# CGuerreroCordova/HydroDEM

Measured on AMD Instinct MI355X. Metric: Mcells/s sink-fill+D8 on 16384^2 float32 DEM, higher is better.
Workload: dtype f32; 1 GPU; 16384x16384 float32 synthetic DEM (SURVEY 8d 'rough': plane + 4 sinusoids + 0.5 m noise + 0.1% pits), SinkFill eps=0 to exact convergence + D8; 16384 rows per GPU, row-block partition; rows_per_gpu=16384, cols=16384, tiles=70225, visits_unchanged=25936, visits_flat=3302, certifying_rounds=0, halo_exchanges=0

## Files before the change

hydrodem_amd/csrc/hdem_sinkfill.hip:

```cpp
#include "hdem_internal.h"

#include <algorithm>
#include <cmath>
#include <cstdlib>

namespace {

constexpr int FT = 62;
constexpr int WN = 64;
constexpr int TS = WN + 1;
constexpr int NT = 64;
constexpr int ITER_MAX = 8;
constexpr int INIT_NT = 256;
constexpr int INIT_ROWS = 4;
constexpr int KEY_NONE = 0x7fffffff;
constexpr int SEED_KEYS = 1 << 20;
constexpr int AUX_SC1 = 16;
constexpr int COARSE_SHIFT = 4;
constexpr int HUB_EDGE = 4 * WN;
constexpr float HUB_BIG = 3.0e38f;
constexpr int HUB_MIN_TILES = 64;
constexpr int HUB_MIN_TILES_NESTED = 36;
constexpr int COARSE_MIN_CELLS = 6000 * 6000;
constexpr int PEND_SHARDS = 64;
// ... 11 lines not shown
constexpr int HEAD_INTS = 32;
constexpr int FLAT_NONE = 0x7f7f7f7f;
enum { ST_IDLE = 0, ST_QUEUED = 1, ST_RUNNING = 2, ST_DIRTY = 3, ST_ROUND0 = 16 };

struct fill_ws {
    int *tile_key;
    int *state;
    int *prio;
    int *pend;
    int *any;
    int *error;
    unsigned long long *stats;
    int *flat;
    int *zmax;
    int *applied;
    int ntiles, tiles_x, tiles_y, max_rounds, G, S;
};

__device__ __forceinline__ float lane_prev(float v)
{
    return __builtin_bit_cast(float, __builtin_amdgcn_update_dpp(
        0, __builtin_bit_cast(int, v), 0x138, 0xF, 0xF, true));
}
__device__ __forceinline__ float lane_next(float v)
{
    return __builtin_bit_cast(float, __builtin_amdgcn_update_dpp(
        0, __builtin_bit_cast(int, v), 0x130, 0xF, 0xF, true));
}

__device__ __forceinline__ void or_changed(unsigned long long &acc, float a, float b)
{
    asm volatile("v_cmp_neq_f32 vcc, %1, %2\n\ts_or_b64 %0, %0, vcc"
                 : "+s"(acc) : "v"(a), "v"(b) : "vcc", "scc");
}
__device__ __forceinline__ void or_less(unsigned long long &acc, float a, float b)
{
    asm volatile("v_cmp_lt_f32 vcc, %1, %2\n\ts_or_b64 %0, %0, vcc"
                 : "+s"(acc) : "v"(a), "v"(b) : "vcc", "scc");
}

__device__ __forceinline__ void shift_in_less(unsigned &acc, float a, float b)
{
    asm volatile("v_cmp_lt_f32 vcc, %1, %2\n\t"
                 "v_addc_co_u32 %0, vcc, %0, %0, vcc"
                 : "+v"(acc) : "v"(a), "v"(b) : "vcc");
}

__device__ __forceinline__ void column_bits(unsigned &west, unsigned &east, float a, float b,
                                            int shift)
{
    unsigned t;
    asm volatile("v_cmp_lt_f32 vcc, %3, %4\n\t"
                 "s_and_b32 %2, vcc_lo, 1\n\t"
                 "s_lshl_b32 %2, %2, %5\n\t"
                 "s_or_b32 %0, %0, %2\n\t"
                 "s_lshr_b32 %2, vcc_hi, 31\n\t"
                 "s_lshl_b32 %2, %2, %5\n\t"
                 "s_or_b32 %1, %1, %2"
                 : "+s"(west), "+s"(east), "=&s"(t)
                 : "v"(a), "v"(b), "i"(shift)
                 : "vcc", "scc");
}

struct scan_masks {
    unsigned long long first, last, all;
};

template <bool HAS_EPS>
__device__ __forceinline__ void scan_lines(const float (&z)[WN], float (&w)[WN], float eps)
{
    float pf = w[0], pb = w[WN - 1];
    asm volatile("s_nop 1" : "+v"(pf), "+v"(pb));
#pragma unroll
    for (int k = 1; k <= WN - 2; ++k) {
        const int i = k, j = WN - 1 - k;
        float t1, t2, cf, cb, nf, nb;
        if (HAS_EPS)
            asm("v_min_f32_dpp %0, %6, %6 wave_shr:1 row_mask:0xf bank_mask:0xf bound_ctrl:0\n\t"
                "v_min_f32_dpp %1, %7, %7 wave_shr:1 row_mask:0xf bank_mask:0xf bound_ctrl:0\n\t"
                "v_min_f32_dpp %2, %6, %0 wave_shl:1 row_mask:0xf bank_mask:0xf bound_ctrl:0\n\t"
                "v_min_f32_dpp %3, %7, %1 wave_shl:1 row_mask:0xf bank_mask:0xf bound_ctrl:0\n\t"
                "v_add_f32 %2, %2, %12\n\t"
                "v_add_f32 %3, %3, %12\n\t"
                "v_med3_f32 %4, %8, %9, %2\n\t"
                "v_med3_f32 %5, %10, %11, %3"
                : "=&v"(t1), "=&v"(t2), "=&v"(cf), "=&v"(cb), "=&v"(nf), "=&v"(nb)
                : "v"(pf), "v"(pb), "v"(z[i]), "v"(w[i]), "v"(z[j]), "v"(w[j]), "v"(eps));
        else
            asm("v_min_f32_dpp %0, %6, %6 wave_shr:1 row_mask:0xf bank_mask:0xf bound_ctrl:0\n\t"
                "v_min_f32_dpp %1, %7, %7 wave_shr:1 row_mask:0xf bank_mask:0xf bound_ctrl:0\n\t"
                "v_min_f32_dpp %2, %6, %0 wave_shl:1 row_mask:0xf bank_mask:0xf bound_ctrl:0\n\t"
                "v_min_f32_dpp %3, %7, %1 wave_shl:1 row_mask:0xf bank_mask:0xf bound_ctrl:0\n\t"
                "v_med3_f32 %4, %8, %9, %2\n\t"
                "v_med3_f32 %5, %10, %11, %3"
                : "=&v"(t1), "=&v"(t2), "=&v"(cf), "=&v"(cb), "=&v"(nf), "=&v"(nb)
                : "v"(pf), "v"(pb), "v"(z[i]), "v"(w[i]), "v"(z[j]), "v"(w[j]));
        w[i] = nf;
        pf = nf;
        w[j] = nb;
        pb = nb;
    }
}

template <bool HAS_EPS>
__device__ __forceinline__ void check_rows(const float (&z)[WN], float (&w)[WN], float eps,
                                           scan_masks &m)
{
    float h_prev = fminf(fminf(w[0], lane_prev(w[0])), lane_next(w[0]));
    float h_cur = fminf(fminf(w[1], lane_prev(w[1])), lane_next(w[1]));
#pragma unroll
    for (int r = 1; r <= WN - 2; ++r) {
        const float h_next = fminf(fminf(w[r + 1], lane_prev(w[r + 1])), lane_next(w[r + 1]));
        float c = fminf(fminf(h_prev, h_cur), h_next);
        if (HAS_EPS) c = c + eps;
        const float n = __builtin_amdgcn_fmed3f(z[r], w[r], c);
        if (r == 1) or_changed(m.first, n, w[r]);
        else if (r == WN - 2) or_changed(m.last, n, w[r]);
        else or_changed(m.all, n, w[r]);
        w[r] = n;
        h_prev = h_cur;
        h_cur = h_next;
    }
}

__device__ __forceinline__ void transpose(float (&v)[WN], float *T, int lane)
{
#pragma unroll
    for (int i = 0; i < WN; ++i) T[i * TS + lane] = v[i];
    __syncthreads();
#pragma unroll
    for (int i = 0; i < WN; ++i) v[i] = T[lane * TS + i];
    __syncthreads();
}

__device__ __forceinline__ float wave_min(float v)
{
#pragma unroll
    for (int o = 32; o >= 1; o >>= 1) v = fminf(v, __shfl_xor(v, o));
    return v;
}

__device__ __forceinline__ int float_key(float f)
{
    int i = __builtin_bit_cast(int, f);
    return i ^ ((i >> 31) & 0x7fffffff);
}

#ifdef HDEM_VISIT_PROF
#define PROF_MARK(k) do { long long now_ = wall_clock64(); out.ticks[k] += now_ - tprof_; tprof_ = now_; } while (0)
#else
#define PROF_MARK(k) do { } while (0)
#endif

struct hub_bounds {
    float lv[9];
    bool mine;
};

struct visit_result {
#ifdef HDEM_VISIT_PROF
    long long ticks[6];
#endif
    bool changed;
    bool more;
    unsigned dirs;
    int iters;
    int flat_bits;
    int zmax_bits;
};

template <bool HAS_EPS, bool COHERENT>
__device__ __forceinline__ visit_result tile_visit(const float *__restrict__ zg, float *wg,
                                                   int H, int W, float eps, int ty, int tx,
                                                   float *T, uint8_t *d8 = nullptr,
                                                   float flat_level = HDEM_INF,
                                                   const hub_bounds *hb = nullptr)
{
    const int lane = threadIdx.x;
    const int y0 = ty * FT, x0 = tx * FT;
    const int x = x0 + lane;
#ifdef HDEM_VISIT_PROF
    const long long tprof_entry_ = wall_clock64();
#endif

    float z[WN], w[WN];
    const int xc = min(x, W - 1);
    float *wbase = wg + (size_t)y0 * W;
    const size_t wbytes = (size_t)(H - y0) * W * sizeof(float);
    const __amdgpu_buffer_rsrc_t wrsrc = __builtin_amdgcn_make_buffer_rsrc(
        wbase, 0, COHERENT ? (int)(unsigned)(wbytes < 0xffffffffull ? wbytes : 0xffffffffull) : 0,
        0x00020000);
    const int hbrow = H - 1 - y0;
    if (COHERENT) {
        const __amdgpu_buffer_rsrc_t zrsrc = __builtin_amdgcn_make_buffer_rsrc(
            const_cast<float *>(zg) + (size_t)y0 * W, 0,
            (int)(unsigned)(wbytes < 0xffffffffull ? wbytes : 0xffffffffull), 0x00020000);
        const unsigned col = (unsigned)xc * (unsigned)sizeof(float);
        const unsigned pitch = (unsigned)W * (unsigned)sizeof(float);
#pragma unroll
        for (int r = 0; r < WN; ++r) {
            const unsigned row = (unsigned)min(r, hbrow) * pitch;
            z[r] = __builtin_bit_cast(float, __builtin_amdgcn_raw_buffer_load_b32(zrsrc, col, row, 0));
            w[r] = __builtin_bit_cast(float, __builtin_amdgcn_raw_buffer_load_b32(wrsrc, col, row, AUX_SC1));
        }
    } else {
#pragma unroll
        for (int r = 0; r < WN; ++r) {
            const size_t o = (size_t)min(y0 + r, H - 1) * W + xc;
            z[r] = zg[o];
            w[r] = wg[o];
        }
    }
    const bool lane_pin = lane == 0 || lane == WN - 1 || x == 0 || x >= W - 1;
    const bool lane_out = x >= W;
    const bool partial = x0 + WN > W || y0 + WN > H;
    unsigned long long free_n = ~0ull, free_s = ~0ull;
    unsigned free_lo = 0, free_hi = 0;
    float hub_t = -HDEM_INF, hub_m = -HDEM_INF, hub_b = -HDEM_INF;
    if (COHERENT && hb) {
        const int k = lane == 0 ? 0 : (lane == WN - 1 ? 2 : 1);
        hub_t = k == 0 ? hb->lv[0] : (k == 1 ? hb->lv[1] : hb->lv[2]);
        hub_m = k == 0 ? hb->lv[3] : (k == 1 ? hb->lv[4] : hb->lv[5]);
        hub_b = k == 0 ? hb->lv[6] : (k == 1 ? hb->lv[7] : hb->lv[8]);
    }
    const int pin_from = lane_pin ? 0 : min(hbrow, WN - 1);
    const int raise_to = x >= W - 1 ? 0 : min(hbrow, WN);
#pragma unroll
    for (int r = 0; r < WN; ++r) {
        float wc = fminf(w[r], HDEM_INF), zc = fminf(z[r], HDEM_INF);
        if (COHERENT) {
            const float bound = r == 0 ? hub_t : (r == WN - 1 ? hub_b : hub_m);
            wc = fmaxf(wc, r < raise_to ? bound : -HDEM_INF);
        }
        if (!COHERENT && partial && (lane_out || y0 + r >= H)) { wc = HDEM_INF; zc = HDEM_INF; }
        if (COHERENT) {
            if (r == 0) free_n = __ballot(zc < wc);
            if (r == WN - 1) free_s = __ballot(zc < wc);
            if (r < 32) shift_in_less(free_lo, zc, wc);
            else shift_in_less(free_hi, zc, wc);
        }
        z[r] = (r == 0 || r == WN - 1 || r >= pin_from) ? wc : zc;
        w[r] = wc;
    }
    if (COHERENT && partial) {
        const unsigned long long in_lanes = __ballot(!lane_out);
        free_n &= in_lanes;
        free_s = hbrow >= WN - 1 ? (free_s & in_lanes) : 0ull;
    }

    if (COHERENT && flat_level < HDEM_INF) {
        const bool inner_lane = lane >= 2 && lane <= FT - 1;
#pragma unroll
        for (int r = 2; r <= FT - 1; ++r) w[r] = inner_lane ? flat_level : w[r];
    }

    unsigned long long free_w = 0, free_e = 0;
    if (COHERENT) {
        const unsigned wl = __builtin_amdgcn_readlane(free_lo, 0), wh = __builtin_amdgcn_readlane(free_hi, 0);
        const unsigned el = __builtin_amdgcn_readlane(free_lo, WN - 1), eh = __builtin_amdgcn_readlane(free_hi, WN - 1);
        free_w = ((unsigned long long)__builtin_bitreverse32(wh) << 32) | __builtin_bitreverse32(wl);
        free_e = ((unsigned long long)__builtin_bitreverse32(eh) << 32) | __builtin_bitreverse32(el);
        if (partial && hbrow < WN - 1) {
            const unsigned long long in_rows = (2ull << hbrow) - 1;
            free_w &= in_rows;
            free_e &= in_rows;
        }
    }
    visit_result out;
    out.flat_bits = out.zmax_bits = FLAT_NONE;
#ifdef HDEM_VISIT_PROF
    for (int k = 0; k < 6; ++k) out.ticks[k] = 0;
    long long tprof_ = tprof_entry_;
    asm volatile("s_waitcnt vmcnt(0)" ::: "memory");
    PROF_MARK(0);
#endif
    out.dirs = 0;
    out.iters = 0;
    scan_masks V = {0, 0, 0};
    check_rows<HAS_EPS>(z, w, eps, V);
    V.all |= V.first | V.last;
    bool more = V.all != 0;
    out.changed = more;
    const bool force_store = COHERENT && hb && hb->mine;
    const unsigned long long b1 = 1ull << 1, bl = 1ull << FT;
    unsigned long long mv_r1 = V.first, mv_r62 = V.last, mv_c1 = V.all & b1, mv_c62 = V.all & bl;
    PROF_MARK(1);
    if (more || force_store) {
        float zt[WN];
#pragma unroll
        for (int r = 0; r < WN; ++r) zt[r] = z[r];
        transpose(zt, T, lane);
        float r1_prev = w[1], r62_prev = w[FT];
        if (lane == 1 || lane == FT) {
            float *dst = T + (lane == 1 ? 0 : WN);
#pragma unroll
            for (int r = 0; r < WN; ++r) dst[r] = w[r];
        }
        __syncthreads();
        float c1_prev = T[lane], c62_prev = T[WN + lane];
        __syncthreads();
        float hl = HDEM_INF, hr = HDEM_INF;
        PROF_MARK(2);
        for (; out.iters < ITER_MAX && more; ++out.iters) {
            scan_lines<HAS_EPS>(z, w, eps);
            transpose(w, T, lane);
            hl = w[0];
            hr = w[WN - 1];
            or_changed(mv_c1, w[1], c1_prev);
            or_changed(mv_c62, w[FT], c62_prev);
            c1_prev = w[1];
            c62_prev = w[FT];
            scan_lines<HAS_EPS>(zt, w, eps);
            or_changed(mv_c1, w[1], c1_prev);
            or_changed(mv_c62, w[FT], c62_prev);
            c1_prev = w[1];
            c62_prev = w[FT];
#pragma unroll
            for (int i = 0; i < WN; ++i) T[lane * TS + i] = w[i];
            __syncthreads();
#pragma unroll
            for (int i = 0; i < WN; ++i) w[i] = T[i * TS + lane];
            __syncthreads();
            or_changed(mv_r1, w[1], r1_prev);
            or_changed(mv_r62, w[FT], r62_prev);
            scan_masks c = {0, 0, 0};
            check_rows<HAS_EPS>(z, w, eps, c);
            c.all |= c.first | c.last;
            mv_r1 |= c.first;
            mv_r62 |= c.last;
            mv_c1 |= c.all & b1;
            mv_c62 |= c.all & bl;
            r1_prev = w[1];
            r62_prev = w[FT];
            more = c.all != 0;
        }

        PROF_MARK(3);
        if (lane >= 1 && lane <= FT && x <= W - 2) {
#pragma unroll
            for (int r = 1; r <= FT; ++r) {
                const int y = y0 + r;
                if (y <= H - 2) {
                    const float val = z[r] == HDEM_INF ? __builtin_nanf("") : w[r];
                    if (COHERENT)
                        __builtin_amdgcn_raw_buffer_store_b32(
                            __builtin_bit_cast(unsigned, val), wrsrc,
                            (unsigned)(((size_t)r * W + x) * sizeof(float)), 0, AUX_SC1);
                    else
                        wg[(size_t)y * W + x] = val;
                }
            }
        }

#ifdef HDEM_VISIT_PROF
        asm volatile("s_waitcnt vmcnt(0)" ::: "memory");
#endif
        PROF_MARK(4);
        const unsigned long long mid = ((1ull << FT) - 1) << 1;
        const bool inner = lane >= 1 && lane <= FT;
        const float e1 = inner ? w[1] : HDEM_INF, e62 = inner ? w[FT] : HDEM_INF;
        const float p1s = lane_prev(e1), n1s = lane_next(e1);
        const float p62s = lane_prev(e62), n62s = lane_next(e62);
        const float p1 = lane == 0 ? HDEM_INF : p1s;
        const float n1 = lane == WN - 1 ? HDEM_INF : n1s;
        const float p62 = lane == 0 ? HDEM_INF : p62s;
        const float n62 = lane == WN - 1 ? HDEM_INF : n62s;
        float cn = fminf(fminf(e1, p1), n1), cs = fminf(fminf(e62, p62), n62);
        if (HAS_EPS) { cn += eps; cs += eps; }
        unsigned long long north = 0, south = 0;
        or_less(north, cn, w[0]);
        or_less(south, cs, w[WN - 1]);
        north &= free_n;
        south &= free_s;
        const bool row1_moved = mv_r1 != 0, row62_moved = mv_r62 != 0;
        if (row1_moved) {
            if (north & mid) out.dirs |= 1u << 1;
            if (north & 1ull) out.dirs |= 1u << 0;
            if (north & (1ull << (WN - 1))) out.dirs |= 1u << 2;
        }
        if (row62_moved) {
            if (south & mid) out.dirs |= 1u << 6;
            if (south & 1ull) out.dirs |= 1u << 5;
            if (south & (1ull << (WN - 1))) out.dirs |= 1u << 7;
        }
        const bool col1_moved = mv_c1 != 0, col62_moved = mv_c62 != 0;
        if (more) {
            if (col1_moved) out.dirs |= 1u << 3;
            if (col62_moved) out.dirs |= 1u << 4;
        } else if (col1_moved || col62_moved) {
            const float m1 = inner ? c1_prev : HDEM_INF, m62 = inner ? c62_prev : HDEM_INF;
            const float pws = lane_prev(m1), nxs = lane_next(m1);
            const float pes = lane_prev(m62), nes = lane_next(m62);
            const float pw = lane == 0 ? HDEM_INF : pws;
            const float nx = lane == WN - 1 ? HDEM_INF : nxs;
            const float pe = lane == 0 ? HDEM_INF : pes;
            const float ne = lane == WN - 1 ? HDEM_INF : nes;
            float cwest = fminf(fminf(m1, pw), nx), ceast = fminf(fminf(m62, pe), ne);
            if (HAS_EPS) { cwest += eps; ceast += eps; }
            unsigned long long west = 0, east = 0;
            or_less(west, cwest, hl);
            or_less(east, ceast, hr);
            if (COHERENT) {
                west &= free_w;
                east &= free_e;
            }
            if (col1_moved && (west & mid)) out.dirs |= 1u << 3;
            if (col62_moved && (east & mid)) out.dirs |= 1u << 4;
        }
        PROF_MARK(5);
    }
    if (COHERENT && !HAS_EPS && !partial && !more) {
        const bool inner_lane = lane >= 1 && lane <= FT;
        const float level = __builtin_bit_cast(
            float, __builtin_amdgcn_readlane(__builtin_bit_cast(int, w[31]), 31));
        if ((__ballot(inner_lane && w[31] != level) == 0) && level < HDEM_INF) {
            unsigned long long off = 0;
            float zm = -HDEM_INF;
#pragma unroll
            for (int r = 1; r <= FT; ++r) {
                or_changed(off, w[r], level);
                zm = fmaxf(zm, z[r]);
            }
            if ((off & ((((1ull << FT) - 1) << 1))) == 0) {
                zm = inner_lane ? zm : -HDEM_INF;
                zm = -wave_min(-zm);
                out.flat_bits = __builtin_bit_cast(int, level);
                out.zmax_bits = __builtin_bit_cast(int, zm);
            }
        }
    }
    if (!COHERENT && d8 && !out.changed) {
        const bool mine = lane >= 1 && lane <= FT && x <= W - 2;
        const float dg = 0.70710678f;
        float nw = lane_prev(w[0]), ne = lane_next(w[0]);
        float cw = lane_prev(w[1]), ce = lane_next(w[1]);
#pragma unroll
        for (int r = 1; r <= FT; ++r) {
            const float sw = lane_prev(w[r + 1]), se = lane_next(w[r + 1]);
            const float c = w[r];
            float best = 0.0f, d;
            unsigned code = 0;
            d = (c - nw) * dg;   if (d > best) { best = d; code = 32; }
            d = (c - w[r - 1]);  if (d > best) { best = d; code = 64; }
            d = (c - ne) * dg;   if (d > best) { best = d; code = 128; }
            d = (c - cw);        if (d > best) { best = d; code = 16; }
            d = (c - ce);        if (d > best) { best = d; code = 1; }
            d = (c - sw) * dg;   if (d > best) { best = d; code = 8; }
            d = (c - w[r + 1]);  if (d > best) { best = d; code = 4; }
            d = (c - se) * dg;   if (d > best) { best = d; code = 2; }
            if (z[r] == HDEM_INF) code = 0;
            const int y = y0 + r;
            if (mine && y <= H - 2) d8[(size_t)y * W + x] = (uint8_t)code;
            nw = cw; ne = ce; cw = sw; ce = se;
        }
    }
    out.more = more;
    return out;
}

__device__ __forceinline__ int neighbour_tile(int k, int ty, int tx, int tiles_x, int tiles_y)
{
    const int dy = k < 3 ? -1 : (k < 5 ? 0 : 1);
    const int dx = (k == 0 || k == 3 || k == 5) ? -1 : ((k == 1 || k == 6) ? 0 : 1);
    const int ny = ty + dy, nx = tx + dx;
    return (ny >= 0 && ny < tiles_y && nx >= 0 && nx < tiles_x) ? ny * tiles_x + nx : -1;
}

__device__ __forceinline__ void add_stats(unsigned long long *stats, int b, bool changed,
                                          bool more, int iters)
{
    unsigned long long *s = stats + (size_t)b * STAT_WORDS;
    s[0] += 1;
    s[1] += (unsigned long long)iters;
    s[2] += changed ? 0 : 1;
    s[3] += more ? 1 : 0;
}

template <bool HAS_EPS>
__global__ __launch_bounds__(NT, 2) void fill_round_kernel(const float *__restrict__ zg,
                                                          float *wg, int H, int W, float eps,
                                                          int tiles_x, int tiles_y, int ntiles,
                                                          int S, int *state, int stamp,
                                                          int *any_next,
                                                          unsigned long long *stats,
                                                          uint8_t *d8)
{
    __shared__ float T[WN * TS];
    const int lane = threadIdx.x;
    const int G = gridDim.x, b = blockIdx.x;
    int *my_state = state + (size_t)b * S;
    for (int base = 0; base < S; base += NT) {
        const int slot_l = base + lane;
        const bool due_l = slot_l < S && slot_l * G + b < ntiles && my_state[slot_l] == stamp;
        unsigned long long due = __ballot(due_l);
        while (due) {
            const int slot = base + __builtin_ctzll(due);
            due &= due - 1;
            const int t = slot * G + b;
            const int ty = t / tiles_x, tx = t - ty * tiles_x;
            visit_result v = tile_visit<HAS_EPS, false>(zg, wg, H, W, eps, ty, tx, T, d8);
            if (d8 && v.changed) { v.dirs = 0xffu; v.more = true; }
            if (lane < 8 && ((v.dirs >> lane) & 1u)) {
                const int t2 = neighbour_tile(lane, ty, tx, tiles_x, tiles_y);
                if (t2 >= 0) {
                    state[(size_t)(t2 % G) * S + t2 / G] = stamp + 1;
                    *any_next = 1;
                }
            }
            if (lane == 8) {
                if (v.more) {
                    my_state[slot] = stamp + 1;
                    *any_next = 1;
                }
                add_stats(stats, b, v.changed, v.more, v.iters);
                stats[(size_t)b * STAT_WORDS + 6] += 1;
#ifdef HDEM_VISIT_PROF
                for (int k = 0; k < 6; ++k) stats[(size_t)b * STAT_WORDS + STAT_PROF + k] += v.ticks[k];
#endif
            }
        }
    }
}

__device__ __forceinline__ int ld_relaxed(const int *p)
{
    return __hip_atomic_load(p, __ATOMIC_RELAXED, __HIP_MEMORY_SCOPE_AGENT);
}

__device__ __forceinline__ void wake_async(int t2, int key, int G, int S, int *state,
                                           int *prio, int *pend)
{
    const int owner = t2 % G, idx = owner * S + t2 / G;
    atomicMin(&prio[idx], key);
    for (int tries = 0; tries < 8; ++tries) {
        const int s = atomicCAS(&state[idx], ST_IDLE, ST_QUEUED);
        if (s == ST_IDLE) {
            atomicAdd(pend + (owner % PEND_SHARDS) * PEND_STRIDE, 1);
            return;
        }
        if (s == ST_QUEUED || s == ST_DIRTY) return;
        const int s2 = atomicCAS(&state[idx], ST_RUNNING, ST_DIRTY);
        if (s2 != ST_IDLE) return;
    }
}

__device__ __attribute__((noinline)) int async_pick(int b, int G, int S, int ntiles, int *state,
                                                    int *prio, const int *pend, int *error,
                                                    long long t_begin, long long budget_ticks)
{
    const int lane = threadIdx.x;
    int *my_state = state + (size_t)b * S, *my_prio = prio + (size_t)b * S;
    int zero_reads = 0;
    for (;;) {
        long long best = 0x7fffffffffffffffll;
        for (int base = 0; base < S; base += NT) {
            const int slot = base + lane;
            long long cand = 0x7fffffffffffffffll;
            if (slot < S && slot * G + b < ntiles && ld_relaxed(&my_state[slot]) == ST_QUEUED)
                cand = ((long long)ld_relaxed(&my_prio[slot]) << 32) | (unsigned)slot;
            best = cand < best ? cand : best;
        }
#pragma unroll
        for (int o = 32; o >= 1; o >>= 1) {
            const long long other = __shfl_xor(best, o);
            best = other < best ? other : best;
        }
        if (best != 0x7fffffffffffffffll) {
            const int slot = (int)(best & 0xffffffffll);
            int got = 0;
            if (lane == 0) got = atomicCAS(&my_state[slot], ST_QUEUED, ST_RUNNING) == ST_QUEUED;
            got = __shfl(got, 0);
            if (!got) continue;
            if (lane == 0) atomicExch(&my_prio[slot], KEY_NONE);
            return slot * G + b;
        }
        for (int tries = 0; tries < 4; ++tries) {
            const int victim = (int)((unsigned)(b + 1 + (unsigned)(wall_clock64() >> 3) % (unsigned)G +
                                                tries * 997u) % (unsigned)G);
            const int *vs = state + (size_t)victim * S;
            int found = -1;
            for (int base = 0; base < S && found < 0; base += NT) {
                const int slot = base + lane;
                const bool q = slot < S && slot * G + victim < ntiles &&
                               ld_relaxed(&vs[slot]) == ST_QUEUED;
                const unsigned long long m = __ballot(q);
                if (m) found = base + __builtin_ctzll(m);
            }
            if (found >= 0) {
                int got = 0;
                if (lane == 0)
                    got = atomicCAS(&state[(size_t)victim * S + found], ST_QUEUED, ST_RUNNING) ==
                          ST_QUEUED;
                got = __shfl(got, 0);
                if (got) {
                    if (lane == 0) atomicExch(&prio[(size_t)victim * S + found], KEY_NONE);
                    return found * G + victim;
                }
            }
        }
        int p = ld_relaxed(&pend[lane * PEND_STRIDE]);
#pragma unroll
        for (int o = 32; o >= 1; o >>= 1) p += __shfl_xor(p, o);
        if (p <= 0) { if (++zero_reads >= 2) return -1; } else zero_reads = 0;
        if (wall_clock64() - t_begin > budget_ticks) {
            if (lane == 0) atomicCAS(error, 0, 1);
            return -1;
        }
        if (ld_relaxed(error) != 0) return -1;
        __builtin_amdgcn_s_sleep(32);
    }
}

__device__ __attribute__((noinline)) void async_finish(int t, int b, int G, int S, int tiles_x,
                                                       int tiles_y, int *state, int *prio,
                                                       int *pend, unsigned long long *stats,
                                                       bool changed, bool more, unsigned dirs,
                                                       int iters)
{
    const int lane = threadIdx.x;
    const int ty = t / tiles_x, tx = t - ty * tiles_x, slot = t / G, owner = t % G;
    int *my_state = state + (size_t)owner * S, *my_prio = prio + (size_t)owner * S;
    const int now_key = SEED_KEYS + (int)(wall_clock64() & 0x3fffffff);
    if (changed && dirs) {
        asm volatile("s_waitcnt vmcnt(0)" ::: "memory");
        if (lane < 8 && ((dirs >> lane) & 1u)) {
            const int t2 = neighbour_tile(lane, ty, tx, tiles_x, tiles_y);
            if (t2 >= 0) wake_async(t2, now_key, G, S, state, prio, pend);
        }
    }
    if (lane == 8) {
        if (more) atomicMin(&my_prio[slot], now_key);
        const int target = more ? ST_QUEUED : ST_IDLE;
        const int old = atomicCAS(&my_state[slot], ST_RUNNING, target);
        if (old == ST_DIRTY) atomicExch(&my_state[slot], ST_QUEUED);
        else if (target == ST_IDLE) atomicAdd(pend + (owner % PEND_SHARDS) * PEND_STRIDE, -1);
        add_stats(stats, b, changed, more, iters);
    }
}

struct flat_result {
    int handled;
    bool changed;
    unsigned dirs;
    float level;
};

__device__ __attribute__((noinline)) flat_result flat_visit(float *wg, int H, int W, int ty, int tx,
                                                            float L, float zmax,
                                                            const hub_bounds *hb)
{
    const int lane = threadIdx.x;
    const int y0 = ty * FT, x0 = tx * FT;
    float *wbase = wg + (size_t)y0 * W;
    const size_t wbytes = (size_t)(H - y0) * W * sizeof(float);
    const __amdgpu_buffer_rsrc_t wrsrc = __builtin_amdgcn_make_buffer_rsrc(
        wbase, 0, (int)(unsigned)(wbytes < 0xffffffffull ? wbytes : 0xffffffffull), 0x00020000);
    auto at = [&](int r, int c) { return (unsigned)(((size_t)r * W + x0 + c) * sizeof(float)); };
    auto ld = [&](unsigned off) {
        return fminf(__builtin_bit_cast(float, __builtin_amdgcn_raw_buffer_load_b32(
                         wrsrc, off, 0, AUX_SC1)), HDEM_INF);
    };
    float top = ld(at(0, lane)), bottom = ld(at(WN - 1, lane));
    float left = ld(at(lane, 0)), right = ld(at(lane, WN - 1));
    if (hb) {
        const int k = lane == 0 ? 0 : (lane == WN - 1 ? 2 : 1);
        top = fmaxf(top, k == 0 ? hb->lv[0] : (k == 1 ? hb->lv[1] : hb->lv[2]));
        bottom = fmaxf(bottom, k == 0 ? hb->lv[6] : (k == 1 ? hb->lv[7] : hb->lv[8]));
        left = fmaxf(left, k == 0 ? hb->lv[0] : (k == 1 ? hb->lv[3] : hb->lv[6]));
        right = fmaxf(right, k == 0 ? hb->lv[2] : (k == 1 ? hb->lv[5] : hb->lv[8]));
    }
    const float low = wave_min(fminf(fminf(top, bottom), fminf(left, right)));
    flat_result out = {1, false, 0u, L};
    if (low >= L) return out;
    if (low < zmax) { out.handled = 0; return out; }
    out.changed = true;
    out.level = low;
    const unsigned bits = __builtin_bit_cast(unsigned, low);
    if (lane >= 1 && lane <= FT) {
        __builtin_amdgcn_raw_buffer_store_b32(bits, wrsrc, at(1, lane), 0, AUX_SC1);
        __builtin_amdgcn_raw_buffer_store_b32(bits, wrsrc, at(FT, lane), 0, AUX_SC1);
        if (lane >= 2 && lane <= FT - 1) {
            __builtin_amdgcn_raw_buffer_store_b32(bits, wrsrc, at(lane, 1), 0, AUX_SC1);
            __builtin_amdgcn_raw_buffer_store_b32(bits, wrsrc, at(lane, FT), 0, AUX_SC1);
        }
    }
    const unsigned long long mid = ((1ull << FT) - 1) << 1, hi = 1ull << (WN - 1);
    const unsigned long long n = __ballot(top > low), s_ = __ballot(bottom > low);
    const unsigned long long w_ = __ballot(left > low), e = __ballot(right > low);
    if (n & 1ull) out.dirs |= 1u << 0;
    if (n & mid) out.dirs |= 1u << 1;
    if (n & hi) out.dirs |= 1u << 2;
    if (w_ & mid) out.dirs |= 1u << 3;
    if (e & mid) out.dirs |= 1u << 4;
    if (s_ & 1ull) out.dirs |= 1u << 5;
    if (s_ & mid) out.dirs |= 1u << 6;
    if (s_ & hi) out.dirs |= 1u << 7;
    return out;
}

__global__ __launch_bounds__(NT) void flat_store_kernel(float *wg, int H, int W, int tiles_x,
                                                        int ntiles, const int *__restrict__ flat,
                                                        const float *__restrict__ hub_lev,
                                                        const int *__restrict__ applied,
                                                        const int *__restrict__ seam_words)
{
    const int t = blockIdx.x;
    if (t >= ntiles) return;
    if (seam_words && (seam_words[0] | seam_words[1] | seam_words[2]) == 0) return;
    const int ty = t / tiles_x, tx = t - ty * tiles_x;
    const int lane = threadIdx.x;
    if (hub_lev && !applied[t]) {
        float l = hub_lev[(size_t)(2 * ty + 1) * (2 * tiles_x + 1) + 2 * tx + 1];
        if (l >= HUB_BIG) l = HDEM_INF;
        const int x = tx * FT + lane;
        if (l == l && lane >= 1 && lane <= FT && x <= W - 2) {
            float *p = wg + (size_t)(ty * FT + 1) * W + x;
            for (int r = 1; r <= FT && ty * FT + r <= H - 2; ++r, p += W) {
                const float v = *p;
                if (v == v) *p = fmaxf(v, l);
            }
        }
        return;
    }
    if (flat[t] == FLAT_NONE) return;
    const float level = __builtin_bit_cast(float, flat[t]);
    if (lane < 2 || lane > FT - 1) return;
    float *p = wg + (size_t)(ty * FT + 2) * W + tx * FT + lane;
    for (int r = 2; r <= FT - 1; ++r, p += W) *p = level;
}


template <int ITERS>
__global__ __launch_bounds__(NT, 2) void hub_dist_kernel(const float *__restrict__ zg,
                                                        float *__restrict__ wg, int H, int W,
                                                        int tiles_x, int ntiles,
                                                        float *__restrict__ edge,
                                                        float *__restrict__ node)
{
    __shared__ float T[WN * TS];
    const int lane = threadIdx.x;
    const int per = (ntiles + 7) / 8;
    for (int b = blockIdx.x; b < 8 * per; b += gridDim.x) {
    const int t = (b & 7) * per + (b >> 3);
    if (t >= ntiles) continue;
    const int ty = t / tiles_x, tx = t - ty * tiles_x;
    const int y0 = ty * FT, x0 = tx * FT, x = x0 + lane, xc = min(x, W - 1);
    float z[WN], w[WN];
    const int hbrow = H - 1 - y0;
    const unsigned pitch = (unsigned)W * (unsigned)sizeof(float), col = (unsigned)xc * (unsigned)sizeof(float);
    const size_t zbytes = (size_t)min(hbrow + 1, WN) * pitch, dbytes = (size_t)min(hbrow, WN) * pitch;
    const __amdgpu_buffer_rsrc_t zrsrc = __builtin_amdgcn_make_buffer_rsrc(
        const_cast<float *>(zg) + (size_t)y0 * W, 0, (int)(unsigned)zbytes, 0x00020000);
    const __amdgpu_buffer_rsrc_t drsrc = __builtin_amdgcn_make_buffer_rsrc(
        wg + (size_t)y0 * W, 0, (int)(unsigned)dbytes, 0x00020000);
#pragma unroll
    for (int r = 0; r < WN; ++r)
        z[r] = __builtin_bit_cast(float, __builtin_amdgcn_raw_buffer_load_b32(
            zrsrc, col, (unsigned)r * pitch, 0));
    float zsum = 0.0f;
#pragma unroll
    for (int r = 0; r < WN; ++r) zsum += z[r];
    const bool nan_any = __ballot(zsum != zsum) != 0;
    const int lr = min(FT, H - 2 - y0), lc = min(FT, W - 2 - x0);
    const bool lane_in = lane >= 1 && lane <= lc;
    const int row_in = lane_in ? lr : 0;
    bool outlet = false;
#pragma unroll
    for (int r = 0; r < WN; ++r) w[r] = HDEM_INF;
    if (nan_any) {
        auto near_row = [&](float v) {
            const float n = v != v ? 1.0f : 0.0f;
            return fmaxf(fmaxf(n, lane_prev(n)), lane_next(n));
        };
        float h_prev = near_row(z[0]), h_cur = near_row(z[1]), any = 0.0f;
#pragma unroll
        for (int r = 1; r <= FT; ++r) {
            const float h_next = near_row(z[r + 1]);
            const bool src = r <= row_in && fmaxf(fmaxf(h_prev, h_cur), h_next) > 0.0f && z[r] == z[r];
            w[r] = src ? z[r] : HDEM_INF;
            any = src ? 1.0f : any;
            h_prev = h_cur;
            h_cur = h_next;
        }
        outlet = __ballot(any != 0.0f) != 0;
    }
    z[0] = z[WN - 1] = HDEM_INF;
#pragma unroll
    for (int r = 1; r <= FT; ++r) z[r] = r <= row_in ? fminf(z[r], HDEM_INF) : HDEM_INF;
    float hz = HDEM_INF;
    if (!outlet) {
        float m = HDEM_INF;
#pragma unroll
        for (int r = 1; r <= FT; ++r) m = fminf(m, z[r]);
        hz = wave_min(m);
        const int L = __builtin_ctzll(__ballot(m == hz) | (1ull << 63));
        int rr = 0;
#pragma unroll
        for (int r = FT; r >= 1; --r) rr = z[r] == hz ? r : rr;
        rr = lane == L ? rr : -1;
#pragma unroll
        for (int r = 1; r <= FT; ++r) w[r] = rr == r ? hz : HDEM_INF;
    }
    float zt[WN];
#pragma unroll
    for (int r = 0; r < WN; ++r) zt[r] = z[r];
    transpose(zt, T, lane);
    float col_w = HDEM_INF, col_e = HDEM_INF;
#pragma unroll
    for (int k = 0; k < ITERS; ++k) {
        scan_lines<false>(z, w, 0.0f);
        transpose(w, T, lane);
        scan_lines<false>(zt, w, 0.0f);
        if (k == ITERS - 1) {
            col_w = w[1];
            col_e = w[FT];
            if (lc != FT) {
#pragma unroll
                for (int i = 1; i < FT; ++i) col_e = i == lc ? w[i] : col_e;
            }
        }
#pragma unroll
        for (int i = 0; i < WN; ++i) T[lane * TS + i] = w[i];
        __syncthreads();
#pragma unroll
        for (int i = 0; i < WN; ++i) w[i] = T[i * TS + lane];
        __syncthreads();
    }
    float row_s = w[FT];
    if (lr != FT) {
#pragma unroll
        for (int i = 1; i < FT; ++i) row_s = i == lr ? w[i] : row_s;
    }
    float *e = edge + (size_t)t * HUB_EDGE;
    e[lane] = w[1];
    e[WN + lane] = row_s;
    e[2 * WN + lane] = col_w;
    e[3 * WN + lane] = col_e;
    if (lane == 0) node[t] = outlet ? __builtin_nanf("") : hz;
    if (lane_in) {
#pragma unroll
        for (int r = 1; r <= FT; ++r)
            __builtin_amdgcn_raw_buffer_store_b32(
                __builtin_bit_cast(unsigned, z[r] == HDEM_INF ? __builtin_nanf("") : w[r]), drsrc,
                col, (unsigned)r * pitch, 0);
    }
    }
}

__device__ __forceinline__ float seam_cost(float a, float b, int lane)
{
    const float p = lane_prev(b), n = lane_next(b);
    const float edge = (lane == 0 || lane == WN - 1) ? HDEM_INF : a;
    return wave_min(fmaxf(edge, fminf(fminf(p, b), n)));
}

__global__ __launch_bounds__(NT) void hub_edges_kernel(const float *__restrict__ zg,
                                                       float *__restrict__ wg, int H, int W,
                                                       int tiles_x, int tiles_y,
                                                       const float *__restrict__ edge,
                                                       const float *__restrict__ node,
                                                       float *__restrict__ cr, int ghost_top,
                                                       int ghost_bottom)
{
    const int t = blockIdx.x, lane = threadIdx.x;
    const int ty = t / tiles_x, tx = t - ty * tiles_x;
    const int y0 = ty * FT, x0 = tx * FT, cw = 2 * tiles_x + 1;
    const float *e = edge + (size_t)t * HUB_EDGE;
    const float mine_n = e[lane], mine_s = e[WN + lane], mine_w = e[2 * WN + lane],
                mine_e = e[3 * WN + lane];
    auto ring_col = [&](int xr) {
        const int y = y0 + lane;
        if (y > H - 1) return HDEM_INF;
        const float v = zg[(size_t)y * W + xr];
        wg[(size_t)y * W + xr] = v;
        return fminf(v, HDEM_INF);
    };
    auto ring_row = [&](int yr, int ghost) {
        const int xx = x0 + lane;
        if (xx > W - 1) return HDEM_INF;
        if (ghost) {
            const bool out = lane == 0 || lane == WN - 1 || xx == 0 || xx == W - 1;
            return out ? HDEM_INF : fminf(wg[(size_t)yr * W + xx], HDEM_INF);
        }
        const float v = zg[(size_t)yr * W + xx];
        wg[(size_t)yr * W + xx] = v;
        return fminf(v, HDEM_INF);
    };
    auto big = [](float v) { return v < HUB_BIG ? v : HUB_BIG; };
    const float other_e = tx + 1 < tiles_x ? edge[(size_t)(t + 1) * HUB_EDGE + 2 * WN + lane]
                                           : ring_col(W - 1);
    const float other_s = ty + 1 < tiles_y ? edge[(size_t)(t + tiles_x) * HUB_EDGE + lane]
                                           : ring_row(H - 1, ghost_bottom);
    const float ce = seam_cost(mine_e, other_e, lane), cs = seam_cost(mine_s, other_s, lane);
    float cwest = HDEM_INF, cnorth = HDEM_INF;
    if (tx == 0) cwest = seam_cost(mine_w, ring_col(0), lane);
    if (ty == 0) cnorth = seam_cost(mine_n, ring_row(0, ghost_top), lane);
    if (lane == 0) {
        float *row = cr + (size_t)(2 * ty + 1) * cw + 2 * tx + 1;
        const float nz = node[t];
        row[0] = nz != nz ? nz : big(nz);
        row[1] = big(ce);
        row[cw] = big(cs);
        row[cw + 1] = HUB_BIG;
        if (tx == 0) { row[-1] = big(cwest); row[cw - 1] = HUB_BIG; }
        if (ty == 0) { row[-cw] = big(cnorth); row[-cw + 1] = HUB_BIG; }
        if (tx == 0 && ty == 0) row[-cw - 1] = HUB_BIG;
    }
}

template <bool HAS_EPS, int ROLE>
__global__ __launch_bounds__(NT, 2) void fill_async_kernel(const float *__restrict__ zg,
                                                          float *wg, int H, int W, float eps,
                                                          int tiles_x, int tiles_y, int ntiles,
                                                          int S, int *state, int *prio,
                                                          int *pend, int *error,
                                                          unsigned long long *stats,
                                                          long long budget_ticks, int soft,
                                                          int *flat, int *zmax,
                                                          const float *__restrict__ hub_lev,
                                                          int *applied,
                                                          const int *__restrict__ seam_words)
{
    __shared__ float T[WN * TS];
    if (seam_words && (seam_words[0] | seam_words[1] | seam_words[2]) == 0) return;
    const int G = gridDim.x, b = blockIdx.x;
    const long long t_begin = wall_clock64();
    if (threadIdx.x == 0) atomicAdd(error + 1, 1);
    while (ld_relaxed(error + 1) < G && ld_relaxed(error) == 0) {
        if (wall_clock64() - t_begin > 20000) {
            if (threadIdx.x == 0) atomicExch(error + 3, 1);
            break;
        }
        __builtin_amdgcn_s_sleep(8);
    }
    if (ld_relaxed(error) != 0) return;
    long long t_mark = t_begin, busy = 0, idle = 0;
    for (;;) {
        if (soft && wall_clock64() - t_begin > budget_ticks) break;
        const int t = __builtin_amdgcn_readfirstlane(
            async_pick(b, G, S, ntiles, state, prio, pend, soft ? error + 2 : error, t_begin,
                       budget_ticks));
        long long now = wall_clock64();
        idle += now - t_mark;
        t_mark = now;
        if (t < 0) break;
        const int ty = t / tiles_x, tx = t - ty * tiles_x;
        float flat_level = HDEM_INF;
        hub_bounds hb;
        bool use_hb = false, first_visit = false;
        const int fb_raw = HAS_EPS ? FLAT_NONE : ld_relaxed(flat + t);
        if (!HAS_EPS && hub_lev) {
            const int k9 = threadIdx.x < 9 ? (int)threadIdx.x : 4;
            const int ny = ty + k9 / 3 - 1, nx = tx + k9 % 3 - 1;
            const bool there = threadIdx.x < 9 && ny >= 0 && ny < tiles_y && nx >= 0 && nx < tiles_x;
            float l = -HDEM_INF;
            int seen = 1;
            if (there) {
                seen = ld_relaxed(applied + ny * tiles_x + nx);
                l = hub_lev[(size_t)(2 * ny + 1) * (2 * tiles_x + 1) + 2 * nx + 1];
            }
            l = (seen || l != l) ? -HDEM_INF : (l >= HUB_BIG ? HDEM_INF : l);
            first_visit = __builtin_amdgcn_readlane(seen, 4) == 0;
            use_hb = first_visit || __ballot(l > -HDEM_INF) != 0;
            if (use_hb) {
#pragma unroll
                for (int k = 0; k < 9; ++k)
                    hb.lv[k] = __builtin_bit_cast(
                        float, __builtin_amdgcn_readlane(__builtin_bit_cast(int, l), k));
                hb.mine = first_visit;
            }
            asm volatile("" ::: "memory");
        }
        if (!HAS_EPS) {
            const int fb = __builtin_amdgcn_readfirstlane(fb_raw);
            if (fb != FLAT_NONE) {
                flat_level = __builtin_bit_cast(float, fb);
                const float zm = __builtin_bit_cast(
                    float, __builtin_amdgcn_readfirstlane(ld_relaxed(zmax + t)));
                const flat_result f = flat_visit(wg, H, W, ty, tx, flat_level, zm,
                                                 use_hb ? &hb : nullptr);
                if (f.handled) {
                    if (f.changed) {
                        if (threadIdx.x == 0)
                            __hip_atomic_store(flat + t, __builtin_bit_cast(int, f.level),
                                               __ATOMIC_RELAXED, __HIP_MEMORY_SCOPE_AGENT);
                        asm volatile("s_waitcnt vmcnt(0)" ::: "memory");
                    }
                    async_finish(t, b, G, S, tiles_x, tiles_y, state, prio, pend, stats, f.changed,
                                 false, f.dirs, 0);
                    now = wall_clock64();
                    if (threadIdx.x == 8) {
                        stats[(size_t)b * STAT_WORDS + STAT_FLAT] += 1;
                        stats[(size_t)b * STAT_WORDS + STAT_FLAT_SAME] += f.changed ? 0 : 1;
                    }
                    busy += now - t_mark;
                    t_mark = now;
                    continue;
                }
            }
        }
        const visit_result v = tile_visit<HAS_EPS, true>(zg, wg, H, W, eps, ty, tx, T, nullptr,
                                                         flat_level, use_hb ? &hb : nullptr);
        if (first_visit) {
            asm volatile("s_waitcnt vmcnt(0)" ::: "memory");
            if (threadIdx.x == 0)
                __hip_atomic_store(applied + t, 1, __ATOMIC_RELAXED, __HIP_MEMORY_SCOPE_AGENT);
            asm volatile("s_waitcnt vmcnt(0)" ::: "memory");
        }
        if (!HAS_EPS && (v.flat_bits != FLAT_NONE || flat_level < HDEM_INF)) {
            if (threadIdx.x == 0) {
                __hip_atomic_store(flat + t, v.flat_bits, __ATOMIC_RELAXED, __HIP_MEMORY_SCOPE_AGENT);
                if (v.flat_bits != FLAT_NONE)
                    __hip_atomic_store(zmax + t, v.zmax_bits, __ATOMIC_RELAXED,
                                       __HIP_MEMORY_SCOPE_AGENT);
            }
            asm volatile("s_waitcnt vmcnt(0)" ::: "memory");
        }
#ifdef HDEM_VISIT_PROF
        const long long t_v = wall_clock64();
#endif
        async_finish(t, b, G, S, tiles_x, tiles_y, state, prio, pend, stats, v.changed, v.more,
                     v.dirs, v.iters);
        now = wall_clock64();
#ifdef HDEM_VISIT_PROF
        if (threadIdx.x == 8) {
            for (int k = 0; k < 6; ++k) stats[(size_t)b * STAT_WORDS + STAT_PROF + k] += v.ticks[k];
            stats[(size_t)b * STAT_WORDS + STAT_PROF + 6] += (unsigned long long)(now - t_v);
        }
#endif
        busy += now - t_mark;
        t_mark = now;
    }
    if (threadIdx.x == 0) {
        stats[(size_t)b * STAT_WORDS + 4] += (unsigned long long)busy;
        stats[(size_t)b * STAT_WORDS + 5] += (unsigned long long)idle;
    }
}

__global__ __launch_bounds__(INIT_NT) void fill_init_kernel(const float *__restrict__ z,
                                                      float *__restrict__ w, int H, int W,
                                                      int tiles_x, int *tile_key,
                                                      int ghost_top, int ghost_bottom,
                                                      int ghost_given,
                                                      const float *__restrict__ coarse, int cw,
                                                      int shift,
                                                      const int *__restrict__ row_map,
                                                      float level_add)
{
    const int quads = (W + 3) / 4;
    const size_t q = (size_t)blockIdx.x * INIT_NT + threadIdx.x;
    if (q >= (size_t)((H + INIT_ROWS - 1) / INIT_ROWS) * quads) return;
    const int y0 = (int)(q / quads) * INIT_ROWS, x = (int)(q % quads) * 4;
    float v[INIT_ROWS + 2][6];
#pragma unroll
    for (int r = 0; r < INIT_ROWS + 2; ++r) {
        const float *row = z + (size_t)min(max(y0 + r - 1, 0), H - 1) * W;
        v[r][0] = row[max(x - 1, 0)];
        if (x + 4 <= W) {
            const hdem_f4 m = hdem_ld4u(row + x);
            v[r][1] = m[0]; v[r][2] = m[1]; v[r][3] = m[2]; v[r][4] = m[3];
        } else {
#pragma unroll
            for (int k = 0; k < 4; ++k) v[r][1 + k] = row[min(x + k, W - 1)];
        }
        v[r][5] = row[min(x + 4, W - 1)];
    }
#pragma unroll
    for (int rr = 0; rr < INIT_ROWS; ++rr) {
        const int y = y0 + rr;
        if (y >= H) break;
        float level = HDEM_INF;
        if (coarse) {
            level = coarse[(size_t)(row_map ? row_map[y] : (y >> shift)) * cw + (x >> shift)];
            level = level >= 3.0e38f ? HDEM_INF : level + level_add;
        }
        float o[4];
#pragma unroll
        for (int k = 0; k < 4; ++k) {
            const int xx = x + k;
            const float zc = v[rr + 1][1 + k];
            const bool ghost = ((ghost_top && y == 0) || (ghost_bottom && y == H - 1)) &&
                               xx != 0 && xx != W - 1;
            bool pin = y == 0 || y == H - 1 || xx == 0 || xx >= W - 1 || zc != zc;
#pragma unroll
            for (int r = 0; r < 3; ++r)
#pragma unroll
                for (int c = 0; c < 3; ++c) pin |= v[rr + r][k + c] != v[rr + r][k + c];
            if (ghost && ghost_given) {
                const float g = xx < W ? w[(size_t)y * W + xx] : zc;
                o[k] = zc != zc ? zc : fmaxf(g, zc);
                if (zc == zc && g == g && tiles_x > 0 && xx < W) {
                    const int ty = min(max(y - 1, 0), H - 3) / FT, tx = min(max(xx - 1, 0), W - 3) / FT;
                    atomicMin(&tile_key[ty * tiles_x + tx], float_key(o[k]));
                }
            } else if (ghost) {
                o[k] = zc != zc ? zc : fmaxf(level, zc);
            } else {
                o[k] = pin ? zc : fmaxf(level, zc);
                if (pin && zc == zc && tiles_x > 0 && xx < W) {
                    const int ty = min(max(y - 1, 0), H - 3) / FT, tx = min(max(xx - 1, 0), W - 3) / FT;
                    atomicMin(&tile_key[ty * tiles_x + tx], float_key(zc));
                }
            }
        }
        float *dst = w + (size_t)y * W + x;
        if (x + 4 <= W) {
            const hdem_f4 m = {o[0], o[1], o[2], o[3]};
            hdem_st4u(dst, m);
        } else {
#pragma unroll
            for (int k = 0; k < 4; ++k)
                if (x + k < W) dst[k] = o[k];
        }
    }
}

__global__ __launch_bounds__(INIT_NT) void fill_seed_kernel(const int *__restrict__ tile_key,
                                                      int tiles_x, int tiles_y, int H, int mode,
                                                      int G, int S, int async, int *state,
                                                      int *prio, int *pend, int stamp, int *any0,
                                                      const float *__restrict__ coarse, int cw,
                                                      int shift, const int *__restrict__ row_map,
                                                      int W, const float *__restrict__ hub_lev,
                                                      const int *__restrict__ seam_words)
{
    const int t = blockIdx.x * INIT_NT + threadIdx.x;
    if (t >= tiles_x * tiles_y) return;
    if (seam_words && mode > 0) {
        mode &= (seam_words[1] ? HDEM_FILL_ACT_TOP : 0) | (seam_words[2] ? HDEM_FILL_ACT_BOTTOM : 0);
        if (mode == 0) return;
    }
    const int ty = t / tiles_x, tx = t - ty * tiles_x;
    int key = KEY_NONE;
    if (mode < 0) {
        for (int dy = -1; dy <= 1; ++dy)
            for (int dx = -1; dx <= 1; ++dx) {
                const int ny = ty + dy, nx = tx + dx;
                if (ny >= 0 && ny < tiles_y && nx >= 0 && nx < tiles_x)
                    key = min(key, tile_key[ny * tiles_x + nx]);
            }
    } else if (mode == 0 || ((mode & HDEM_FILL_ACT_TOP) && ty == 0) ||
               ((mode & HDEM_FILL_ACT_BOTTOM) && ty == max(H - 3, 0) / FT)) {
        key = 0;
    }
    if (key == KEY_NONE) return;
    const int owner = t % G, idx = owner * S + t / G;
    if (async) {
        if (atomicCAS(&state[idx], ST_IDLE, ST_QUEUED) == ST_IDLE) {
            int k = 0;
            if (hub_lev && mode == 0) {
                const float level = hub_lev[(size_t)(2 * ty + 1) * (2 * tiles_x + 1) + 2 * tx + 1];
                if (level == level)
                    k = min(max((float_key(level) >> 12) + (SEED_KEYS >> 1), 0), SEED_KEYS - 1);
            } else if (coarse && mode == 0) {
                const int y = min(ty * FT + FT / 2, H - 1), x = min(tx * FT + FT / 2, W - 1);
// ... 704 lines not shown
```

Measured before the change: 62190 Mcells/s.

## Prefetch tile Z window before hub-bound and flat-level lookups

In the asynchronous driver, the tile's 64-row Z window is now loaded up front, before the hub-level and flat-level scalar lookups resolve. This lets the Z fetch latency overlap with that bookkeeping. Hub bounds are passed by value as per-lane top/mid/bottom scalars instead of through a pointer to a 9-element array, which removes the branches around them. The cost is that tiles taking the flat_visit path issue a Z load they never use, and a second Z load is issued when flat_visit declines the tile. Register pressure also rises because z is live across the flat_visit call.

```diff
diff --git a/hydrodem_amd/csrc/hdem_sinkfill.hip b/hydrodem_amd/csrc/hdem_sinkfill.hip
--- a/hydrodem_amd/csrc/hdem_sinkfill.hip
+++ b/hydrodem_amd/csrc/hdem_sinkfill.hip
@@ -187,8 +187,8 @@
 #define PROF_MARK(k) do { } while (0)
 #endif
 
-struct hub_bounds {
-    float lv[9];
+struct hub_window {
+    float t, m, b;
     bool mine;
 };
 
@@ -204,12 +204,29 @@
     int zmax_bits;
 };
 
+__device__ __forceinline__ void load_window_z(const float *__restrict__ zg, int H, int W, int ty,
+                                              int tx, float (&z)[WN])
+{
+    const int y0 = ty * FT, xc = min(tx * FT + (int)threadIdx.x, W - 1);
+    const size_t wbytes = (size_t)(H - y0) * W * sizeof(float);
+    const int hbrow = H - 1 - y0;
+    const __amdgpu_buffer_rsrc_t zrsrc = __builtin_amdgcn_make_buffer_rsrc(
+        const_cast<float *>(zg) + (size_t)y0 * W, 0,
+        (int)(unsigned)(wbytes < 0xffffffffull ? wbytes : 0xffffffffull), 0x00020000);
+    const unsigned col = (unsigned)xc * (unsigned)sizeof(float);
+    const unsigned pitch = (unsigned)W * (unsigned)sizeof(float);
+#pragma unroll
+    for (int r = 0; r < WN; ++r) {
+        const unsigned row = (unsigned)min(r, hbrow) * pitch;
+        z[r] = __builtin_bit_cast(float, __builtin_amdgcn_raw_buffer_load_b32(zrsrc, col, row, 0));
+    }
+}
+
 template <bool HAS_EPS, bool COHERENT>
-__device__ __forceinline__ visit_result tile_visit(const float *__restrict__ zg, float *wg,
-                                                   int H, int W, float eps, int ty, int tx,
-                                                   float *T, uint8_t *d8 = nullptr,
-                                                   float flat_level = HDEM_INF,
-                                                   const hub_bounds *hb = nullptr)
+__device__ __forceinline__ visit_result tile_visit_z(const float *__restrict__ zg, float *wg,
+                                                     int H, int W, float eps, int ty, int tx,
+                                                     float *T, float (&z)[WN], uint8_t *d8,
+                                                     float flat_level, const hub_window hub)
 {
     const int lane = threadIdx.x;
     const int y0 = ty * FT, x0 = tx * FT;
@@ -218,7 +235,7 @@
     const long long tprof_entry_ = wall_clock64();
 #endif
 
-    float z[WN], w[WN];
+    float w[WN];
     const int xc = min(x, W - 1);
     float *wbase = wg + (size_t)y0 * W;
     const size_t wbytes = (size_t)(H - y0) * W * sizeof(float);
@@ -227,15 +244,13 @@
         0x00020000);
     const int hbrow = H - 1 - y0;
     if (COHERENT) {
-        const __amdgpu_buffer_rsrc_t zrsrc = __builtin_amdgcn_make_buffer_rsrc(
-            const_cast<float *>(zg) + (size_t)y0 * W, 0,
-            (int)(unsigned)(wbytes < 0xffffffffull ? wbytes : 0xffffffffull), 0x00020000);
         const unsigned col = (unsigned)xc * (unsigned)sizeof(float);
-        const unsigned pitch = (unsigned)W * (unsigned)sizeof(float);
+        unsigned pitch = (unsigned)W * (unsigned)sizeof(float);
+        int last = hbrow;
+        asm("" : "+s"(pitch), "+s"(last));
 #pragma unroll
         for (int r = 0; r < WN; ++r) {
-            const unsigned row = (unsigned)min(r, hbrow) * pitch;
-            z[r] = __builtin_bit_cast(float, __builtin_amdgcn_raw_buffer_load_b32(zrsrc, col, row, 0));
+            const unsigned row = (unsigned)min(r, last) * pitch;
             w[r] = __builtin_bit_cast(float, __builtin_amdgcn_raw_buffer_load_b32(wrsrc, col, row, AUX_SC1));
         }
     } else {
@@ -251,13 +266,7 @@
     const bool partial = x0 + WN > W || y0 + WN > H;
     unsigned long long free_n = ~0ull, free_s = ~0ull;
     unsigned free_lo = 0, free_hi = 0;
-    float hub_t = -HDEM_INF, hub_m = -HDEM_INF, hub_b = -HDEM_INF;
-    if (COHERENT && hb) {
-        const int k = lane == 0 ? 0 : (lane == WN - 1 ? 2 : 1);
-        hub_t = k == 0 ? hb->lv[0] : (k == 1 ? hb->lv[1] : hb->lv[2]);
-        hub_m = k == 0 ? hb->lv[3] : (k == 1 ? hb->lv[4] : hb->lv[5]);
-        hub_b = k == 0 ? hb->lv[6] : (k == 1 ? hb->lv[7] : hb->lv[8]);
-    }
+    const float hub_t = hub.t, hub_m = hub.m, hub_b = hub.b;
     const int pin_from = lane_pin ? 0 : min(hbrow, WN - 1);
     const int raise_to = x >= W - 1 ? 0 : min(hbrow, WN);
 #pragma unroll
@@ -316,7 +325,7 @@
     V.all |= V.first | V.last;
     bool more = V.all != 0;
     out.changed = more;
-    const bool force_store = COHERENT && hb && hb->mine;
+    const bool force_store = COHERENT && hub.mine;
     const unsigned long long b1 = 1ull << 1, bl = 1ull << FT;
     unsigned long long mv_r1 = V.first, mv_r62 = V.last, mv_c1 = V.all & b1, mv_c62 = V.all & bl;
     PROF_MARK(1);
@@ -491,6 +500,17 @@
     }
     out.more = more;
     return out;
+}
+
+template <bool HAS_EPS, bool COHERENT>
+__device__ __forceinline__ visit_result tile_visit(const float *__restrict__ zg, float *wg,
+                                                   int H, int W, float eps, int ty, int tx,
+                                                   float *T, uint8_t *d8 = nullptr)
+{
+    static_assert(!COHERENT, "the asynchronous driver loads Z itself: tile_visit_z");
+    float z[WN];
+    const hub_window none = {-HDEM_INF, -HDEM_INF, -HDEM_INF, false};
+    return tile_visit_z<HAS_EPS, false>(zg, wg, H, W, eps, ty, tx, T, z, d8, HDEM_INF, none);
 }
 
 __device__ __forceinline__ int neighbour_tile(int k, int ty, int tx, int tiles_x, int tiles_y)
@@ -682,7 +702,8 @@
 
 __device__ __attribute__((noinline)) flat_result flat_visit(float *wg, int H, int W, int ty, int tx,
                                                             float L, float zmax,
-                                                            const hub_bounds *hb)
+                                                            float hub_top, float hub_bottom,
+                                                            float hub_left, float hub_right)
 {
     const int lane = threadIdx.x;
     const int y0 = ty * FT, x0 = tx * FT;
@@ -697,13 +718,10 @@
     };
     float top = ld(at(0, lane)), bottom = ld(at(WN - 1, lane));
     float left = ld(at(lane, 0)), right = ld(at(lane, WN - 1));
-    if (hb) {
-        const int k = lane == 0 ? 0 : (lane == WN - 1 ? 2 : 1);
-        top = fmaxf(top, k == 0 ? hb->lv[0] : (k == 1 ? hb->lv[1] : hb->lv[2]));
-        bottom = fmaxf(bottom, k == 0 ? hb->lv[6] : (k == 1 ? hb->lv[7] : hb->lv[8]));
-        left = fmaxf(left, k == 0 ? hb->lv[0] : (k == 1 ? hb->lv[3] : hb->lv[6]));
-        right = fmaxf(right, k == 0 ? hb->lv[2] : (k == 1 ? hb->lv[5] : hb->lv[8]));
-    }
+    top = fmaxf(top, hub_top);
+    bottom = fmaxf(bottom, hub_bottom);
+    left = fmaxf(left, hub_left);
+    right = fmaxf(right, hub_right);
     const float low = wave_min(fminf(fminf(top, bottom), fminf(left, right)));
     flat_result out = {1, false, 0u, L};
     if (low >= L) return out;
@@ -981,39 +999,42 @@
         if (t < 0) break;
         const int ty = t / tiles_x, tx = t - ty * tiles_x;
         float flat_level = HDEM_INF;
-        hub_bounds hb;
-        bool use_hb = false, first_visit = false;
+        bool first_visit = false;
         const int fb_raw = HAS_EPS ? FLAT_NONE : ld_relaxed(flat + t);
-        if (!HAS_EPS && hub_lev) {
-            const int k9 = threadIdx.x < 9 ? (int)threadIdx.x : 4;
-            const int ny = ty + k9 / 3 - 1, nx = tx + k9 % 3 - 1;
-            const bool there = threadIdx.x < 9 && ny >= 0 && ny < tiles_y && nx >= 0 && nx < tiles_x;
-            float l = -HDEM_INF;
-            int seen = 1;
-            if (there) {
-                seen = ld_relaxed(applied + ny * tiles_x + nx);
-                l = hub_lev[(size_t)(2 * ny + 1) * (2 * tiles_x + 1) + 2 * nx + 1];
-            }
-            l = (seen || l != l) ? -HDEM_INF : (l >= HUB_BIG ? HDEM_INF : l);
-            first_visit = __builtin_amdgcn_readlane(seen, 4) == 0;
-            use_hb = first_visit || __ballot(l > -HDEM_INF) != 0;
-            if (use_hb) {
-#pragma unroll
-                for (int k = 0; k < 9; ++k)
-                    hb.lv[k] = __builtin_bit_cast(
-                        float, __builtin_amdgcn_readlane(__builtin_bit_cast(int, l), k));
-                hb.mine = first_visit;
-            }
-            asm volatile("" ::: "memory");
-        }
+        const bool with_hub = !HAS_EPS && hub_lev;
+        const int k9 = threadIdx.x < 9 ? (int)threadIdx.x : 4;
+        const int ny = ty + k9 / 3 - 1, nx = tx + k9 % 3 - 1;
+        const bool there = with_hub && threadIdx.x < 9 && ny >= 0 && ny < tiles_y && nx >= 0 &&
+                           nx < tiles_x;
+        float l = -HDEM_INF;
+        int seen = 1;
+        if (there) {
+            seen = ld_relaxed(applied + ny * tiles_x + nx);
+            l = hub_lev[(size_t)(2 * ny + 1) * (2 * tiles_x + 1) + 2 * nx + 1];
+        }
+        float z[WN];
+        load_window_z(zg, H, W, ty, tx, z);
+        l = (seen || l != l) ? -HDEM_INF : (l >= HUB_BIG ? HDEM_INF : l);
+        if (with_hub) first_visit = __builtin_amdgcn_readlane(seen, 4) == 0;
+        float lv[9];
+#pragma unroll
+        for (int k = 0; k < 9; ++k)
+            lv[k] = __builtin_bit_cast(
+                float, __builtin_amdgcn_readlane(__builtin_bit_cast(int, l), k));
+        const bool lane_lo = threadIdx.x == 0, lane_hi = threadIdx.x == WN - 1;
+        auto pick = [&](int a, int m, int c) {
+            return lane_lo ? lv[a] : (lane_hi ? lv[c] : lv[m]);
+        };
+        const hub_window hub = {pick(0, 1, 2), pick(3, 4, 5), pick(6, 7, 8), first_visit};
+        asm volatile("" ::: "memory");
         if (!HAS_EPS) {
             const int fb = __builtin_amdgcn_readfirstlane(fb_raw);
             if (fb != FLAT_NONE) {
                 flat_level = __builtin_bit_cast(float, fb);
                 const float zm = __builtin_bit_cast(
                     float, __builtin_amdgcn_readfirstlane(ld_relaxed(zmax + t)));
-                const flat_result f = flat_visit(wg, H, W, ty, tx, flat_level, zm,
-                                                 use_hb ? &hb : nullptr);
+                const flat_result f = flat_visit(wg, H, W, ty, tx, flat_level, zm, hub.t, hub.b,
+                                                 pick(0, 3, 6), pick(2, 5, 8));
                 if (f.handled) {
                     if (f.changed) {
                         if (threadIdx.x == 0)
@@ -1032,10 +1053,11 @@
                     t_mark = now;
                     continue;
                 }
+                load_window_z(zg, H, W, ty, tx, z);
             }
         }
-        const visit_result v = tile_visit<HAS_EPS, true>(zg, wg, H, W, eps, ty, tx, T, nullptr,
-                                                         flat_level, use_hb ? &hb : nullptr);
+        const visit_result v = tile_visit_z<HAS_EPS, true>(zg, wg, H, W, eps, ty, tx, T, z, nullptr,
+                                                           flat_level, hub);
         if (first_visit) {
             asm volatile("s_waitcnt vmcnt(0)" ::: "memory");
             if (threadIdx.x == 0)
```

Result: faster. 63350 Mcells/s, median of 6 (+1.9%).
